# zhouhang95/ray_tracing_in_one_weekend

Hardware: AMD Instinct MI355X
Metric: Mray/s (primary+secondary) at 1920x1080/256spp (higher is better)
Workload: dtype f32

## Files before the change

include/rtow_mi355x_debug.h:

```cpp
#ifndef RTOW_MI355X_DEBUG_H
#define RTOW_MI355X_DEBUG_H

#include "rtow_mi355x.h"

#ifdef __cplusplus
extern "C" {
#endif

#define RT_FLAG_TIME_DEPTHS 4u
#define RT_FLAG_PRODUCTION_KERNELS 8u

int rt_get_depth_timings(RtCtx* ctx, uint32_t max_n, float* isect_ms, float* shade_ms, uint64_t* rays);

int rt_debug_render_parts(const RtCtx* ctx, char* buf, uint32_t cap);

enum RtDebugOption {
    RT_OPT_TREE_PLACEMENT = 0,
    RT_OPT_PRIMARY_LISTS = 1,
    RT_OPT_PIXEL_ORDER = 2,
    RT_OPT_TEXEL_POOL = 3,
    RT_OPT_GRID = 4,
    RT_OPT_GRID_CELL = 5,
    RT_OPT_CHAINS = 6,
    RT_OPT_GENERAL_KERNELS = 7,
    RT_OPT_GENERAL_LDS = 8,
    RT_OPT_QUEUE_SHARDS = 9,
    RT_OPT_ISECT_WORKGROUPS = 10,
    RT_OPT_MATERIALISE_PRIMARIES = 11,
    RT_OPT_MEDIUM_SEARCH = 12,
    RT_OPT_POOL_CHUNK_DELAY_US = 13,
    RT_OPT__COUNT = 14
};
int rt_debug_set_option(RtCtx* ctx, uint32_t option, uint32_t value);
int rt_debug_get_option(const RtCtx* ctx, uint32_t option, uint32_t* value);

typedef struct RtSceneInfo {
    uint32_t n_entries;
    uint32_t n_tree_nodes, tree_depth;
    uint32_t tree_in_lds;
    uint32_t general_kernels;
    uint32_t closest_hit_lds_bytes;
    uint32_t grid;
    uint32_t grid_cells[3];
    uint32_t grid_refs;
    uint32_t grid_always;
    uint32_t grid_lds_bytes;
    float grid_cell_size[3];
    uint32_t general_tables_in_lds;
    uint32_t nest;
} RtSceneInfo;
int rt_debug_scene_info(const RtCtx* ctx, RtSceneInfo* info);

int rt_debug_planar_info(const RtCtx* ctx, uint32_t* n_planar, uint32_t* plane_data_in_lds);
int rt_debug_planar_bounds(const RtQuads* quads, float world_mag, float* box, float* slack);

int rt_debug_grid_build(const RtFlatScene* scene, uint32_t cell_per_mille, uint32_t lds_budget, float grid[8], uint32_t dims[3],
                        uint32_t* cells, uint32_t* n_cells, uint16_t* refs, uint32_t* n_refs, uint32_t large[4], uint32_t* n_large);

int rt_debug_world_bounds(const RtFlatScene* scene, float* prim_box, float* prim_box_padded, float* world_sphere, uint32_t* n_entries,
                          uint32_t* entry_id, float* entry_box_padded, float* entry_bs);

int rt_debug_motion_bounds(const RtCtx* ctx, float* entry_box_padded, float* entry_sphere, uint32_t* entry_id, uint32_t entry_cap, uint32_t* n_entries,
                           float grid[6], uint32_t dims[3], uint32_t* cell_begin, uint32_t* cell_id, uint32_t cell_cap, uint32_t* n_cell_ids);

// ... 33 lines not shown
```

ray_tracing_in_one_weekend_amd/_ffi.py:

```python
import ctypes as C
import os

_PKG_DIR = os.path.dirname(os.path.abspath(__file__))
GPU_LIB_PATH = os.environ.get("RTOW_GPU_LIB") or os.path.join(_PKG_DIR, "librtow_mi355x.so")
HOST_LIB_PATH = os.path.join(_PKG_DIR, "librtow_host.so")

RT_NO_TEX = 0xFFFFFFFF
ERR_INVALID, ERR_DEVICE, ERR_NOMEM, ERR_UNSUPPORTED, ERR_STATE = 1, 2, 3, 4, 5
FLAG_BRUTE_FORCE = 1
FLAG_RUSSIAN_ROULETTE = 2
FLAG_TIME_DEPTHS = 4
FLAG_PRODUCTION_KERNELS = 8
RTH_INVALID = 0xFFFFFFFF

(MAT_EMISSION, MAT_DIFFUSE, MAT_LAMBERT, MAT_METAL, MAT_DIELECTRIC, MAT_ISOTROPIC, MAT_OREN_NAYAR,
 MAT_BURLEY_DIFFUSE, MAT_ROUGH_PLASTIC, MAT_DISNEY_DIFFUSE, MAT_DISNEY_METAL, MAT_DISNEY_SHEEN,
 MAT_DISNEY_CLEARCOAT) = range(13)
TEX_CONSTANT, TEX_CHECKER, TEX_PERLIN, TEX_IMAGE = range(4)
RECT_YZ, RECT_XZ, RECT_XY = range(3)
XF_TRANSLATE, XF_ROTATE_Y = range(2)
NO_XFORM = 0xFFFFFFFF
SKY_GRADIENT, SKY_BLACK, SKY_ENV = range(3)

_f = C.POINTER(C.c_float)
# ... 49 lines not shown
PLANAR_MIN_SIN2 = 2.0 ** -20
PLANAR_REACH = 16.0


class RtParams(C.Structure):
    _fields_ = [("nx", C.c_uint32), ("ny", C.c_uint32), ("spp", C.c_uint32), ("max_depth", C.c_int32),
                ("seed", C.c_uint64), ("shard_band", C.c_uint32), ("shard_count", C.c_uint32),
                ("shard_id", C.c_uint32), ("spp_slice", C.c_uint32), ("flags", C.c_uint32), ("reserved", C.c_uint32)]


class RtStats(C.Structure):
    _fields_ = [("n_paths", C.c_uint64), ("n_rays", C.c_uint64), ("n_rays_secondary", C.c_uint64),
                ("n_texture_fetches", C.c_uint64), ("n_bad_dir", C.c_uint64), ("seconds_total", C.c_double),
                ("seconds_trace", C.c_double), ("seconds_device", C.c_double), ("bytes_algorithmic", C.c_uint64),
                ("bytes_trace_algorithmic", C.c_uint64), ("n_trace_launches", C.c_uint32), ("n_slices", C.c_uint32),
                ("rays_per_depth", C.c_uint64 * 64)]

    def as_dict(self):
        d = {k: getattr(self, k) for k, _ in self._fields_ if k != "rays_per_depth"}
        d["rays_per_depth"] = list(self.rays_per_depth)
        return d


class RtBounceIO(C.Structure):
    _fields_ = [("n", C.c_uint32), ("depth", C.c_uint32), ("in_o", _f), ("in_d", _f), ("in_key", _u32),
                ("out_hit", C.POINTER(C.c_int32)), ("out_t", _f), ("out_radiance", _f), ("out_attenuation", _f),
                ("out_o", _f), ("out_d", _f), ("out_alive", _u8), ("flags", C.c_uint32)]


RtProgressFn = C.CFUNCTYPE(None, C.c_void_p, C.c_uint32, C.c_uint32, C.POINTER(C.c_uint8), C.c_uint32, C.c_uint32)

MULTI_COPY_GATHER = 1
(OPT_TREE_PLACEMENT, OPT_PRIMARY_LISTS, OPT_PIXEL_ORDER, OPT_TEXEL_POOL, OPT_GRID, OPT_GRID_CELL, OPT_CHAINS,
 OPT_GENERAL_KERNELS, OPT_GENERAL_LDS, OPT_QUEUE_SHARDS, OPT_ISECT_WORKGROUPS, OPT_MATERIALISE_PRIMARIES, OPT_MEDIUM_SEARCH, OPT_POOL_CHUNK_DELAY_US) = range(14)
OPT_NAMES = {"tree_placement": OPT_TREE_PLACEMENT, "primary_lists": OPT_PRIMARY_LISTS, "pixel_order": OPT_PIXEL_ORDER,
             "texel_pool": OPT_TEXEL_POOL, "grid": OPT_GRID, "grid_cell": OPT_GRID_CELL, "chains": OPT_CHAINS,
             "general_kernels": OPT_GENERAL_KERNELS, "general_lds": OPT_GENERAL_LDS, "queue_shards": OPT_QUEUE_SHARDS,
             "isect_workgroups": OPT_ISECT_WORKGROUPS, "materialise_primaries": OPT_MATERIALISE_PRIMARIES,
             "medium_search": OPT_MEDIUM_SEARCH, "pool_chunk_delay_us": OPT_POOL_CHUNK_DELAY_US}


class RtSceneInfo(C.Structure):
    _fields_ = [("n_entries", C.c_uint32), ("n_tree_nodes", C.c_uint32), ("tree_depth", C.c_uint32), ("tree_in_lds", C.c_uint32),
                ("general_kernels", C.c_uint32), ("closest_hit_lds_bytes", C.c_uint32), ("grid", C.c_uint32),
                ("grid_cells", C.c_uint32 * 3), ("grid_refs", C.c_uint32), ("grid_always", C.c_uint32),
                ("grid_lds_bytes", C.c_uint32), ("grid_cell_size", C.c_float * 3), ("general_tables_in_lds", C.c_uint32), ("nest", C.c_uint32)]

    def as_dict(self):
        d = {k: getattr(self, k) for k, _ in self._fields_ if k not in ("grid_cells", "grid_cell_size")}
        d["grid_cells"], d["grid_cell_size"] = list(self.grid_cells), [float(x) for x in self.grid_cell_size]
        return d


EXPECTED_ABI = 11
GPU_SYMBOLS = ["rt_abi_version", "rt_build_id", "rt_ctx_create", "rt_ctx_destroy", "rt_last_error", "rt_scene_upload",
               "rt_shard_rows", "rt_shard_row_to_image_row", "rt_prepare", "rt_render", "rt_render_device", "rt_debug_bounce", "rt_debug_arithmetic",
               "rt_get_depth_timings", "rt_set_progress", "rt_host_alloc", "rt_host_free", "rt_debug_set_option", "rt_debug_get_option",
               "rt_debug_scene_info", "rt_debug_grid_build", "rt_debug_world_bounds", "rt_debug_render_parts", "rt_multi_create", "rt_multi_create_ex", "rt_multi_destroy", "rt_multi_device_count",
               "rt_multi_last_error", "rt_multi_scene_upload", "rt_multi_render", "rt_deinterleave_bands", "rt_set_lens", "rt_multi_set_lens",
               "rt_set_motion", "rt_multi_set_motion", "rt_debug_motion_bounds",
               "rt_set_quads", "rt_multi_set_quads", "rt_debug_planar_info", "rt_debug_planar_bounds"]
HOST_SYMBOLS = ["rth_last_error", "rth_register_image", "rth_rng_reseed", "rth_scene_build", "rth_scene_new",
                "rth_tex_constant", "rth_tex_checker", "rth_tex_perlin", "rth_tex_image", "rth_material",
                "rth_sphere", "rth_rect", "rth_gbox", "rth_translate", "rth_rotate_y", "rth_constant_medium", "rth_hitable_bbox", "rth_set_sky", "rth_set_camera", "rth_scene_finish", "rth_scene_flat",
                "rth_scene_camera", "rth_scene_sphere_name", "rth_scene_free", "rth_png_write", "rth_output_file_name",
                "rth_set_camera_lens", "rth_scene_lens",
                "rth_moving_sphere", "rth_set_camera_shutter", "rth_scene_motion",
                "rth_quad", "rth_triangle", "rth_scene_quads"]

_gpu_lib = None
_host_lib = None

# ... 181 lines not shown
```

ray_tracing_in_one_weekend_amd/csrc/rt_api.hip:

```cpp
#include "../../include/rtow_mi355x_debug.h"
#include "rt_kernels.h"
#include "rt_bvh.h"
#include "rt_grid.h"
#include "rt_pool.h"

#include <hip/hip_runtime.h>

#include <algorithm>
#include <chrono>
#include <cmath>
#include <cstdio>
#include <cstdlib>
#include <cstring>
#include <new>
#include <string>
#include <vector>

using namespace rt;

namespace {

thread_local std::string g_create_error;

struct DevBuf {
// ... 1431 lines not shown
        gp.s0 = s0;
        gp.n_rays = npix * sc;
        RT_HIP(ctx, hipMemsetAsync(counts, 0, counts_bytes, st));
        if (ctx->motion) hipLaunchKernelGGL(k_set_motion, dim3(1), dim3(64), 0, st, gpd, ctx->gmotion);
        if (ctx->planar) hipLaunchKernelGGL(k_set_planar, dim3(1), dim3(64), 0, st, gpd, ctx->gplanar);
        if (lens) hipLaunchKernelGGL(k_init_counts<true>, dim3((nq + 255u) / 256u), dim3(256), 0, st, gp, counts, gpd, glens);
        else hipLaunchKernelGGL(k_init_counts<false>, dim3((nq + 255u) / 256u), dim3(256), 0, st, gp, counts, gpd, glens);
        if (!fuse_gen && lens) hipLaunchKernelGGL(k_gen_primary<true>, dim3((gp.n_rays + 255u) / 256u), dim3(256), 0, st, gp, Q[0], glens);
        else if (!fuse_gen) hipLaunchKernelGGL(k_gen_primary<false>, dim3((gp.n_rays + 255u) / 256u), dim3(256), 0, st, gp, Q[0], glens);
        RT_HIP(ctx, hipEventRecord(ctx->events[2 * sl], st));
        if (n_groups > 1u) {
            RT_HIP(ctx, hipEventRecord(ctx->ev_fork, st));
            RT_HIP(ctx, hipStreamWaitEvent(ctx->stream2, ctx->ev_fork, 0));
        }
        for (int depth = 0; depth < n_depths; ++depth)
        for (uint32_t grp = 0; grp < n_groups; ++grp) {
            hipStream_t sg = grp ? ctx->stream2 : st;
            const uint32_t q0 = grp * (nq / n_groups), q1 = grp + 1u == n_groups ? nq : q0 + nq / n_groups;
            const uint32_t isect_grid_g = (q1 - q0 + shards_per_wg - 1u) / shards_per_wg;
            const Queue& qi = Q[depth & 1];
            const Queue& qo = Q[(depth + 1) & 1];
            const uint32_t* cin = counts + (size_t)depth * nq;
            uint32_t* cout = counts + (size_t)(depth + 1) * nq;
            const bool td = time_depths && sl == 0;
            if (td) RT_HIP(ctx, hipEventRecord(ctx->depth_events[3 * (size_t)depth], st));
            const bool gen = fuse_gen && depth == 0;
            ip.depth = depth;
            ip.q0 = q0, ip.q1 = q1;
            const StepBuffers sb{qi, qo, qhit, cin, cout, rad, totals, gpd, lens, ctx->motion, ctx->planar};
            const bool no_primary_trace = gen && !rects && gp.lists != nullptr && no_overflow;
            if (!no_primary_trace) launch_intersect(ctx, sg, use_bvh, gen, isect_grid_g, sb, ip);
            if (td) RT_HIP(ctx, hipEventRecord(ctx->depth_events[3 * (size_t)depth + 1], st));
            const ShadeParams sp{nq, cap, depth, prm->max_depth, depth > 0 ? 1u : 0u,
                                 (prm->flags & RT_FLAG_RUSSIAN_ROULETTE) ? 1u : 0u, q0};
            launch_shade(ctx, sg, gen, !rects && gp.lists != nullptr, q1 - q0, sb, sp);
            if (td) RT_HIP(ctx, hipEventRecord(ctx->depth_events[3 * (size_t)depth + 2], st));
            if (grp == 0u) n_trace_launches += no_primary_trace ? 1u : 2u;
        }
        if (n_groups > 1u) {
            RT_HIP(ctx, hipEventRecord(ctx->ev_join, ctx->stream2));
            RT_HIP(ctx, hipStreamWaitEvent(st, ctx->ev_join, 0));
        }
        if (time_depths && sl == 0) {
            ctx->timed_depths = n_depths;
            ctx->timed_rays.assign((size_t)n_depths, 0ull);
            std::vector<uint32_t> hc((size_t)(n_depths + 1) * nq);
            RT_HIP(ctx, hipMemcpyAsync(hc.data(), counts, hc.size() * sizeof(uint32_t), hipMemcpyDeviceToHost, st));
            RT_HIP(ctx, hipStreamSynchronize(st));
            for (int d = 0; d < n_depths; ++d)
                for (uint32_t k = 0; k < nq; ++k) ctx->timed_rays[(size_t)d] += hc[(size_t)d * nq + k];
        }
        RT_HIP(ctx, hipEventRecord(ctx->events[2 * sl + 1], st));
        hipLaunchKernelGGL(k_resolve, dim3((npix + 255u) / 256u), dim3(256), 0, st, rad, acc, npix, sc);
        hipLaunchKernelGGL(k_accum_counts, dim3((unsigned)n_depths), dim3(256), 0, st, counts, nq, (uint32_t)n_depths, totals + 2);
        if (ctx->progress_armed && ctx->progress_fn && s0 + sc < spp) {
            const uint32_t done = s0 + sc;
            hipLaunchKernelGGL(k_finalize, dim3((npix + 255u) / 256u), dim3(256), 0, st, acc, (float*)nullptr,
                               (uint8_t*)ctx->preview_u8.p, nx, rows, done, gp.tiles_per_row, gp.tile_pixels);
            RT_HIP(ctx, hipMemcpyAsync(ctx->preview_host.data(), ctx->preview_u8.p, (size_t)npix * 3, hipMemcpyDeviceToHost, st));
            RT_HIP(ctx, hipStreamSynchronize(st));
            ctx->progress_fn(ctx->progress_user, done, spp, ctx->preview_host.data(), nx, rows);
        }
        s0 += sc;
    }
    if (pool_wait_ms > 0.0) ctx->parts.emplace_back("of_which_waiting_for_the_pool", pool_wait_ms);
    hipLaunchKernelGGL(k_finalize, dim3((npix + 255u) / 256u), dim3(256), 0, st, acc, (float*)d_out_rgb_f32,
                       (uint8_t*)d_out_rgb8, nx, rows, spp, gp.tiles_per_row, gp.tile_pixels);
// ... 673 lines not shown
    if ((rc = ensure(ctx, ctx->counts, (size_t)2 * nq * sizeof(uint32_t)))) return rc;
    if ((rc = ensure(ctx, ctx->totals, 4 * sizeof(unsigned long long)))) return rc;
    if ((rc = ensure(ctx, ctx->genp, sizeof(GenParams) + RT_PLANAR_OFFSET + sizeof(GenPlanar)))) return rc;
    if ((rc = ensure(ctx, ctx->dbg, (size_t)n * 6 * sizeof(float)))) return rc;
    const WorkLayout wl = work_layout((size_t)nq * cap, n);
    const size_t wbase = work_base(ctx);
    if (const char* e = pool_request(ctx->pool, wbase + wl.total)) return fail(ctx, RT_ERR_NOMEM, std::string("rt_debug_bounce: ") + e);
    if (!pool_wait(ctx->pool, wbase + wl.total)) return fail(ctx, RT_ERR_NOMEM, "rt_debug_bounce: no device memory for the work buffers: " + pool_error(ctx->pool));
    const WorkView wv = work_view(ctx, wl, wbase);
    const Queue* Q = wv.Q;
    uint32_t* counts = (uint32_t*)ctx->counts.p;
    float* d_o = (float*)ctx->dbg.p;
    float* d_d = d_o + 3 * (size_t)n;
    RT_HIP(ctx, hipMemcpyAsync(d_o, io->in_o, 3 * (size_t)n * 4, hipMemcpyHostToDevice, st));
    RT_HIP(ctx, hipMemcpyAsync(d_d, io->in_d, 3 * (size_t)n * 4, hipMemcpyHostToDevice, st));
    RT_HIP(ctx, hipMemsetAsync(counts, 0, (size_t)2 * nq * sizeof(uint32_t), st));
    RT_HIP(ctx, hipMemsetAsync(ctx->totals.p, 0, 4 * sizeof(unsigned long long), st));
    RT_HIP(ctx, hipMemsetAsync(wv.rad, 0xFF, (size_t)n * RT_RAD_FLOATS * sizeof(float), st));
    GenParams gp{};
    gp.nx = n, gp.ny = 1, gp.npix = n, gp.n_rays = n, gp.s0 = 0;
    gp.shard_band = 1, gp.shard_count = 1, gp.shard_id = 0;
    gp.nq = nq, gp.cap = cap;
    gp.inv_npix = gp.inv_nx = (float)((1.0 / (double)n) * (1.0 - 1.0 / 4194304.0));
    gp.inv_band = (float)(1.0 - 1.0 / 4194304.0);
    hipLaunchKernelGGL(k_init_counts<false>, dim3((nq + 255u) / 256u), dim3(256), 0, st, gp, counts, (GenParams*)ctx->genp.p, GenLens{});
    if (ctx->motion) hipLaunchKernelGGL(k_set_motion, dim3(1), dim3(64), 0, st, (GenParams*)ctx->genp.p, ctx->gmotion);
    if (ctx->planar) hipLaunchKernelGGL(k_set_planar, dim3(1), dim3(64), 0, st, (GenParams*)ctx->genp.p, ctx->gplanar);
    hipLaunchKernelGGL(k_debug_fill, dim3((n + 255u) / 256u), dim3(256), 0, st, gp, Q[0], d_o, d_d);
    const bool use_bvh = ctx->use_bvh && !(io->flags & RT_FLAG_BRUTE_FORCE);
    const StepBuffers sb{Q[0], Q[1], wv.qhit, counts, counts + nq, wv.rad,
                         (unsigned long long*)ctx->totals.p, (const GenParams*)ctx->genp.p, false, ctx->motion, ctx->planar};
    const IntersectParams ip{nq, cap, (int)io->depth, 0u, nq};
    launch_intersect(ctx, st, use_bvh, false, qg.isect_grid, sb, ip);
    const ShadeParams sp{nq, cap, (int)io->depth, 0x7FFFFFFF, 1u, 0u, 0u};
    launch_shade(ctx, st, false, false, nq, sb, sp);
    RT_HIP(ctx, hipGetLastError());
    std::vector<float4> ha((size_t)nq * cap), hb((size_t)nq * cap);
    std::vector<float> hrad((size_t)n * RT_RAD_FLOATS);
    std::vector<float2> hc((size_t)nq * cap), hh((size_t)nq * cap);
    std::vector<uint32_t> hcnt((size_t)2 * nq);
    RT_HIP(ctx, hipMemcpyAsync(hh.data(), wv.qhit, hh.size() * sizeof(float2), hipMemcpyDeviceToHost, st));
    std::vector<float4> hab;
    if (RT_QSTRIDE == 1u) {
        RT_HIP(ctx, hipMemcpyAsync(ha.data(), Q[1].a, ha.size() * sizeof(float4), hipMemcpyDeviceToHost, st));
        RT_HIP(ctx, hipMemcpyAsync(hb.data(), Q[1].b, hb.size() * sizeof(float4), hipMemcpyDeviceToHost, st));
    } else {
        hab.resize(2 * ha.size());
        RT_HIP(ctx, hipMemcpyAsync(hab.data(), Q[1].a, hab.size() * sizeof(float4), hipMemcpyDeviceToHost, st));
    }
    RT_HIP(ctx, hipMemcpyAsync(hc.data(), Q[1].c, hc.size() * sizeof(float2), hipMemcpyDeviceToHost, st));
    RT_HIP(ctx, hipMemcpyAsync(hrad.data(), wv.rad, hrad.size() * sizeof(float), hipMemcpyDeviceToHost, st));
    RT_HIP(ctx, hipMemcpyAsync(hcnt.data(), counts, hcnt.size() * sizeof(uint32_t), hipMemcpyDeviceToHost, st));
    RT_HIP(ctx, hipStreamSynchronize(st));
    for (size_t i = 0; i < hab.size() / 2; ++i) ha[i] = hab[2 * i], hb[i] = hab[2 * i + 1];
    auto bits = [](float f) {
        uint32_t u;
        std::memcpy(&u, &f, 4);
        return u;
    };
    for (uint32_t i = 0; i < n; ++i) {
        const uint32_t chunk = i >> 8;
        const size_t pos = (size_t)(chunk % nq) * cap + (size_t)(chunk / nq) * 256u + (i & 255u);
        const int hit = (int)bits(hh[pos].y);
        io->out_hit[i] = hit;
        io->out_t[i] = hit >= 0 ? hh[pos].x : 0.0f;
        io->out_alive[i] = 0;
        for (int k = 0; k < 3; ++k) io->out_attenuation[3 * (size_t)i + k] = io->out_o[3 * (size_t)i + k] = io->out_d[3 * (size_t)i + k] = 0.0f;
// ... 125 lines not shown
```

ray_tracing_in_one_weekend_amd/csrc/rt_device.h:

```cpp
#pragma once
#include <hip/hip_runtime.h>
#include <stdint.h>

namespace rt {

struct V3 {
    float x, y, z;
};
struct V2 {
    float x, y;
};
__device__ __forceinline__ V3 v3(float x, float y, float z) { return V3{x, y, z}; }
__device__ __forceinline__ V3 splat(float s) { return V3{s, s, s}; }
__device__ __forceinline__ V3 operator+(V3 a, V3 b) { return V3{a.x + b.x, a.y + b.y, a.z + b.z}; }
__device__ __forceinline__ V3 operator-(V3 a, V3 b) { return V3{a.x - b.x, a.y - b.y, a.z - b.z}; }
__device__ __forceinline__ V3 operator*(V3 a, V3 b) { return V3{a.x * b.x, a.y * b.y, a.z * b.z}; }
__device__ __forceinline__ V3 operator/(V3 a, V3 b) { return V3{a.x / b.x, a.y / b.y, a.z / b.z}; }
__device__ __forceinline__ V3 operator*(V3 a, float s) { return V3{a.x * s, a.y * s, a.z * s}; }
__device__ __forceinline__ V3 operator*(float s, V3 a) { return V3{s * a.x, s * a.y, s * a.z}; }
__device__ __forceinline__ V3 operator/(V3 a, float s) { return V3{a.x / s, a.y / s, a.z / s}; }
__device__ __forceinline__ V3 operator+(V3 a, float s) { return V3{a.x + s, a.y + s, a.z + s}; }
__device__ __forceinline__ V3 operator-(float s, V3 a) { return V3{s - a.x, s - a.y, s - a.z}; }
__device__ __forceinline__ V3 operator-(V3 a) { return V3{-a.x, -a.y, -a.z}; }
__device__ __forceinline__ float dot(V3 a, V3 b) { return (a.x * b.x + a.y * b.y) + a.z * b.z; }
// ... 68 lines not shown
#define RT_LANE_STAT(I, PRED)                                                                      \
    do {                                                                                           \
        const unsigned long long act_ = __ballot(true), m_ = __ballot(PRED);                       \
        if ((threadIdx.x & 63u) == (uint32_t)__ffsll((long long)act_) - 1u) {                      \
            atomicAdd(&g_lane_stats[I], 64ull);                                                    \
            atomicAdd(&g_lane_stats[(I) + 1], (unsigned long long)__popcll(m_));                   \
        }                                                                                          \
    } while (0)
#else
#define RT_LANE_STAT(I, PRED)
#endif

__device__ __forceinline__ uint32_t fmix32(uint32_t h) {
    h ^= h >> 16;
    h *= 0x85EBCA6Bu;
    h ^= h >> 13;
    h *= 0xC2B2AE35u;
    h ^= h >> 16;
    return h;
}
__device__ __forceinline__ uint32_t mix32(uint32_t h) {
    h ^= h >> 16;
    h *= 0x7FEB352Du;
    h ^= h >> 15;
    h *= 0x846CA68Bu;
    h ^= h >> 16;
    return h;
}
__device__ __forceinline__ void path_key(uint64_t seed, uint32_t pix, uint32_t samp, uint32_t& k0, uint32_t& k1) {
    uint32_t s_lo = (uint32_t)seed, s_hi = (uint32_t)(seed >> 32);
    uint32_t a = fmix32(pix ^ s_lo);
    k0 = fmix32(a + samp * 0x9E3779B9u + s_hi);
    k1 = fmix32((a ^ 0xA511E9B3u) + samp * 0xC2B2AE3Du);
}
struct Rng {
    uint32_t k0, k1, w;
    __device__ __forceinline__ Rng() {}
    __device__ __forceinline__ Rng(uint32_t k0_, uint32_t k1_, uint32_t ctr) : k0(k0_), k1(k1_), w(ctr * 0x9E3779B9u) {}
    __device__ __forceinline__ float next() {
        uint32_t r = mix32((k0 ^ w) + k1);
        w += 0x9E3779B9u;
        return (float)(r >> 8) * (1.0f / 16777216.0f);
    }
    __device__ __forceinline__ float next_pm1() {
        uint32_t r = mix32((k0 ^ w) + k1);
        w += 0x9E3779B9u;
        return __builtin_fmaf((float)(r >> 8), 1.0f / 8388608.0f, -1.0f);
    }
};
__device__ __forceinline__ uint32_t depth_counter_base(int depth) { return (uint32_t)(depth + 1) * 256u; }

__device__ __forceinline__ V3 random_in_unit_sphere(Rng& rng) {
    RT_LANE_STAT(10, true);
    for (;;) {
        RT_LANE_STAT(8, true);
        const float x = rng.next_pm1();
        const float y = rng.next_pm1();
        const float z = rng.next_pm1();
        const V3 v = v3(x, y, z);
        if (length_squared(v) < 1.0f) return v;
    }
}
__device__ __forceinline__ V3 random_on_hemisphere(Rng& rng, V3 n) {
    V3 v = random_in_unit_sphere(rng);
    if (!(dot(v, n) > 0.0f)) v = -v;
    return normalize(v);
// ... 278 lines not shown
    V3 oc = o - v3(g.x, g.y, g.z);
    float half_b = dot(oc, d);
    float c = length_squared(oc) - g.w * g.w;
    if (t_min > 0.0f && half_b > 0.0f && c > 0.0f) return false;
    float discriminant = half_b * half_b - a * c;
    if (discriminant < 0.0f) return false;
    float sqrtd = sqrt_ns(discriminant);
    float root = (-half_b - sqrtd) / a;
    if (root < t_min || t_max < root) {
        root = (-half_b + sqrtd) / a;
        if (root < t_min || t_max < root) return false;
    }
    t_hit = root;
    return true;
}

__device__ __forceinline__ bool sphere_root(float4 g, V3 o, V3 d, const SharedRcp& ra, float t_min, float t_max, float& t_hit) {
    V3 oc = o - v3(g.x, g.y, g.z);
    float half_b = dot(oc, d);
    float c = length_squared(oc) - g.w * g.w;
    if (half_b > 0.0f && c > 0.0f) return false;
    float discriminant = half_b * half_b - ra.a * c;
    if (discriminant < 0.0f) return false;
    float sqrtd = sqrt_ns(discriminant);
    float root = div_shared(-half_b - sqrtd, ra);
    if (root < t_min || t_max < root) {
        root = div_shared(-half_b + sqrtd, ra);
        if (root < t_min || t_max < root) return false;
    }
    t_hit = root;
    return true;
}

__device__ __forceinline__ bool rect_root(float4 g0, float4 g1, V3 o, V3 d, float t_min, float t_max, float& t_hit) {
    const uint32_t axis = __float_as_uint(g1.y);
    const float oa = axis == 0u ? o.x : (axis == 1u ? o.y : o.z);
    const float da = axis == 0u ? d.x : (axis == 1u ? d.y : d.z);
    const float t = (g0.x - oa) / da;
    if (!(t == t) || t < t_min || t > t_max) return false;
    const V3 p = o + d * t;
    const float pu = axis == 0u ? p.y : p.x;
    const float pv = axis == 2u ? p.y : p.z;
    if (pu < g0.y || pu > g0.z || pv < g0.w || pv > g1.x) return false;
    t_hit = t;
    return true;
}

#define RT_PLANAR_TRIANGLE_DEV 1u
__device__ __forceinline__ void planar_coords(const float4* __restrict__ g, V3 P, float& alpha, float& beta) {
    const float4 q4 = g[1], u4 = g[2], v4 = g[3], w4 = g[4];
    const V3 p = P - v3(q4.x, q4.y, q4.z);
    const V3 w = v3(w4.x, w4.y, w4.z);
    alpha = dot(w, cross(p, v3(v4.x, v4.y, v4.z)));
    beta = dot(w, cross(v3(u4.x, u4.y, u4.z), p));
}
__device__ __forceinline__ bool planar_root(const float4* __restrict__ g, V3 o, V3 d, float t_min, float t_max, float& t_hit) {
    const float4 nd = g[0];
    const V3 normal = v3(nd.x, nd.y, nd.z);
    const float denom = dot(normal, d);
    if (fabsf(denom) < 1e-8f) return false;
    const float t = (nd.w - dot(normal, o)) / denom;
    if (!(t == t) || t < t_min || t > t_max) return false;
    const V3 P = o + d * t;
    float alpha, beta;
    planar_coords(g, P, alpha, beta);
    const bool inside = __float_as_uint(g[1].w) == RT_PLANAR_TRIANGLE_DEV ? (alpha >= 0.0f && beta >= 0.0f && alpha + beta <= 1.0f)
// ... 371 lines not shown
```

ray_tracing_in_one_weekend_amd/csrc/rt_kernels.h:

```cpp
#pragma once
#include "rt_device.h"

namespace rt {

#ifndef RT_QSTRIDE
#define RT_QSTRIDE 2u
#endif
struct Queue {
    float4* a;
    float4* b;
    float2* c;
};
#ifndef RT_RAD_FLOATS
#define RT_RAD_FLOATS 3
#endif
__device__ __forceinline__ void rad_store(float* __restrict__ rad, size_t slot, float x, float y, float z) {
    if (RT_RAD_FLOATS == 4) *reinterpret_cast<float4*>(rad + 4u * slot) = make_float4(x, y, z, 0.0f);
    else *reinterpret_cast<float3*>(rad + 3u * slot) = make_float3(x, y, z);
}

struct GenParams {
    float cam_origin[3], cam_horizontal[3], cam_vertical[3], cam_llc[3];
    uint32_t nx, ny;
    uint32_t npix;
// ... 97 lines not shown
    Rng rng;
    path_key(((uint64_t)gp.seed_hi << 32) | gp.seed_lo, j * gp.nx + i, samp, rng.k0, rng.k1);
    rng.w = 0u;
    const float u = ((float)i + rng.next()) / (float)gp.nx;
    const float v = ((float)j + rng.next()) / (float)gp.ny;
    const V3 origin = v3(gp.cam_origin[0], gp.cam_origin[1], gp.cam_origin[2]);
    const V3 H = v3(gp.cam_horizontal[0], gp.cam_horizontal[1], gp.cam_horizontal[2]);
    const V3 Vv = v3(gp.cam_vertical[0], gp.cam_vertical[1], gp.cam_vertical[2]);
    const V3 llc = v3(gp.cam_llc[0], gp.cam_llc[1], gp.cam_llc[2]);
    o = origin;
    if (!LENS) {
        d = normalize(llc + u * H + v * Vv - origin);
    } else {
        const V3 dir = llc + u * H + v * Vv - origin;
        float rx = 0.0f, ry = 0.0f;
        for (uint32_t t = 0; t < RT_LENS_TRIPS; ++t) {
            const float x = rng.next_pm1(), y = rng.next_pm1();
            if (x * x + y * y < 1.0f) {
                rx = x, ry = y;
                break;
            }
        }
        const V3 off = rx * v3(gl.lu[0], gl.lu[1], gl.lu[2]) + ry * v3(gl.lv[0], gl.lv[1], gl.lv[2]);
        o = origin + off;
        d = normalize(gl.focus_dist * dir - off);
    }
    k0 = rng.k0, k1 = rng.k1;
}
template <bool LENS>
__device__ __forceinline__ void gen_primary(const GenParams& gp, const GenLens& gl, uint32_t idx, V3& o, V3& d, uint32_t& k0,
                                            uint32_t& k1) {
    uint32_t pl;
    gen_primary<LENS>(gp, gl, idx, o, d, k0, k1, pl);
}

__device__ __forceinline__ uint32_t primary_idx_of(uint32_t nq, uint32_t shard, uint32_t pos) {
    return ((pos >> 8) * nq + shard) * 256u + (pos & 255u);
}
template <bool LENS>
__global__ __launch_bounds__(256) void k_init_counts(GenParams gp, uint32_t* __restrict__ counts,
                                                     GenParams* __restrict__ gp_dev, GenLens gl) {
    const uint32_t sq = blockIdx.x * 256u + threadIdx.x;
    if (sq == 0) *gp_dev = gp;
    if (LENS && sq == 0) *reinterpret_cast<GenLens*>(gp_dev + 1) = gl;
    if (sq >= gp.nq) return;
    const uint32_t nchunks = (gp.n_rays + 255u) / 256u;
    const uint32_t nc = sq < nchunks ? (nchunks - sq + gp.nq - 1u) / gp.nq : 0u;
    uint32_t cnt = nc * 256u;
    if (nc && ((nchunks - 1u) % gp.nq) == sq) cnt -= nchunks * 256u - gp.n_rays;
    counts[sq] = cnt;
}

__global__ void k_set_motion(GenParams* __restrict__ gp_dev, GenMotion gm) {
    if (blockIdx.x == 0 && threadIdx.x == 0) *reinterpret_cast<GenMotion*>(reinterpret_cast<char*>(gp_dev + 1) + RT_MOTION_OFFSET) = gm;
}

__global__ void k_set_planar(GenParams* __restrict__ gp_dev, GenPlanar pl) {
    if (blockIdx.x == 0 && threadIdx.x == 0) *reinterpret_cast<GenPlanar*>(reinterpret_cast<char*>(gp_dev + 1) + RT_PLANAR_OFFSET) = pl;
}

template <bool LENS>
__global__ __launch_bounds__(256) void k_gen_primary(GenParams gp, Queue q, GenLens gl) {
    const uint32_t idx = blockIdx.x * 256u + threadIdx.x;
    if (idx >= gp.n_rays) return;
    V3 o, d;
    uint32_t k0, k1;
// ... 818 lines not shown
            tbest = th;
            hit = (int)(gq.base + i);
        }
    }
}

__global__ __launch_bounds__(256) void k_intersect_list_planar(DevScene sc, const float4* __restrict__ qa, const float4* __restrict__ qb,
                                                               float2* __restrict__ qh, const uint32_t* __restrict__ in_counts,
                                                               IntersectParams ip, const GenParams* __restrict__ gpd) {
    const uint32_t q = ip.q0 + blockIdx.x;
    const uint32_t count = in_counts[q];
    const size_t qbase = (size_t)q * ip.cap;
    const GenPlanar gq = gen_planar_of(gpd);
    for (uint32_t i = threadIdx.x; i < count; i += 256u) {
        const float4 ra = qa[RT_QSTRIDE * (qbase + i)], rb = qb[RT_QSTRIDE * (qbase + i)];
        const V3 o = v3(ra.x, ra.y, ra.z), d = v3(rb.x, rb.y, rb.z);
        float tbest = RT_FLT_MAX;
        int hit = -1;
        closest_hit_spheres_general(sc, o, d, tbest, hit);
        MediumCtx mc{0u, 0u, depth_counter_base(ip.depth)};
        if (sc.n_media) path_key_of_slot(*gpd, __float_as_uint(ra.w), mc.k0, mc.k1);
        closest_hit_rects(sc, o, d, mc, tbest, hit);
        closest_hit_planar(gq, o, d, tbest, hit);
        qh[qbase + i] = make_float2(tbest, __int_as_float(hit));
    }
}

struct ShadeParams {
    uint32_t nq, cap;
    int depth, max_depth;
    uint32_t sort;
    uint32_t russian_roulette;
    uint32_t q0;
};

#ifdef RT_PROFILE_PHASES
__device__ unsigned long long g_phase_stats[16];
#define RT_PHASE_CLOCK() __builtin_amdgcn_s_memtime()
#else
#define RT_PHASE_CLOCK() 0ull
#endif

#define RT_PERLIN_LDS_MAX_SETS 4u
#ifndef RT_SORT_N
#define RT_SORT_N 512u
#endif
#define RT_NCLASS 64u
#define RT_CLASS_LDS_MAX 4096u
#define RT_SHADE_WAVE_LDS (RT_NCLASS * 4u + RT_SORT_N * 8u + RT_SORT_N * 2u)
__host__ __device__ inline size_t shade_lds_bytes(uint32_t n_entries, uint32_t n_perlin_lds, uint32_t n_fused_spheres, bool sort) {
    size_t b = 16u;
    if (sort) b += 4u * RT_SHADE_WAVE_LDS;
    if (sort && n_entries <= RT_CLASS_LDS_MAX) b += ((size_t)n_entries + 15u) & ~(size_t)15u;
    b += (size_t)n_perlin_lds * (4096u + 1536u);
    b += (size_t)n_fused_spheres * 16u;
    return (b + 15u) & ~(size_t)15u;
}
template <bool PERLIN_LDS, bool GEN, bool RECTS, bool NEST = false, bool LENS = false, bool MOTION = false, bool PLANAR = false>
#ifndef RT_GEN_WAVES
#define RT_GEN_WAVES 4
#endif
#ifndef RT_SORTED_WAVES
#define RT_SORTED_WAVES 4
#endif
__global__ __launch_bounds__(256, GEN ? RT_GEN_WAVES : RT_SORTED_WAVES) void k_shade(DevScene sc, Queue qin, const float2* __restrict__ qh, Queue qout,
                                               const uint32_t* __restrict__ in_counts, uint32_t* __restrict__ out_counts,
// ... 3 lines not shown
    extern __shared__ __attribute__((aligned(16))) char smem[];
    const uint32_t q = tp.q0 + blockIdx.x;
    const uint32_t count = in_counts[q];
    if (count == 0) return;
    uint32_t* s_out = reinterpret_cast<uint32_t*>(smem);
    const uint32_t lane = threadIdx.x & 63u;
    const uint32_t w = __builtin_amdgcn_readfirstlane(threadIdx.x >> 6);
    const bool sort = !GEN && tp.sort != 0u;
    size_t lds_off = 16u;
    uint32_t* s_hist = reinterpret_cast<uint32_t*>(smem + lds_off + (size_t)w * RT_SHADE_WAVE_LDS);
    float2* s_rec = reinterpret_cast<float2*>(s_hist + RT_NCLASS);
    unsigned short* s_pos = reinterpret_cast<unsigned short*>(s_rec + RT_SORT_N);
    const uint8_t* cls = sc.sph_class;
    if (sort) {
        lds_off += 4u * RT_SHADE_WAVE_LDS;
        const uint32_t n_ent = sc.n_prims + sc.n_media + (PLANAR ? gen_planar_of(gpd).n : 0u);
        if (n_ent <= RT_CLASS_LDS_MAX) {
            uint8_t* lc = reinterpret_cast<uint8_t*>(smem + lds_off);
            for (uint32_t i = threadIdx.x; i < n_ent; i += 256u) lc[i] = sc.sph_class[i];
            cls = lc;
            lds_off += ((size_t)n_ent + 15u) & ~(size_t)15u;
        }
    }
    PerlinTables pt{sc.perlin_vec, sc.perlin_perm2};
    if (PERLIN_LDS) {
        float4* lv = reinterpret_cast<float4*>(smem + lds_off);
        unsigned short* lp = reinterpret_cast<unsigned short*>(lv + sc.n_perlin * 256u);
        for (uint32_t i = threadIdx.x; i < sc.n_perlin * 256u; i += 256u) lv[i] = sc.perlin_vec[i];
        for (uint32_t i = threadIdx.x; i < sc.n_perlin * 768u; i += 256u) lp[i] = sc.perlin_perm2[i];
        pt = PerlinTables{lv, lp};
        lds_off += (size_t)sc.n_perlin * (4096u + 1536u);
    }
    const bool fused = GEN && !RECTS && gpd->lists != nullptr;
    const float4* s_geo = reinterpret_cast<const float4*>(smem + lds_off);
    if (fused) {
        float4* g = reinterpret_cast<float4*>(smem + lds_off);
        for (uint32_t i = threadIdx.x; i < sc.n_spheres; i += 256u) g[i] = sc.sph_geo[i];
        if (MOTION)
            for (uint32_t i = threadIdx.x; i < sc.n_spheres; i += 256u) g[sc.n_spheres + i] = gen_motion_of(gpd).sph_dc[i];
    }
    const float4* s_dc = s_geo + sc.n_spheres;
    if (threadIdx.x == 0) *s_out = 0u;
    __syncthreads();
    uint32_t n_fetch = 0, n_bad = 0;
    const size_t qbase = (size_t)q * tp.cap;
#ifdef RT_PROFILE_PHASES
    unsigned long long ph[10] = {};
    const unsigned long long ph_t0 = RT_PHASE_CLOCK();
#endif
    const uint32_t bs = count >= 4u * RT_SORT_N ? RT_SORT_N : ((count + 255u) / 256u) * 64u;
    for (uint32_t base = w * bs; base < count; base += 4u * bs) {
        const uint32_t n_here = min(bs, count - base);
#ifdef RT_PROFILE_PHASES
        const unsigned long long ph_a0 = RT_PHASE_CLOCK();
        asm volatile("s_waitcnt vmcnt(0)" ::: "memory");
        const unsigned long long ph_a = RT_PHASE_CLOCK();
        ph[8] += ph_a - ph_a0;
#endif
        if (sort) {
            s_hist[lane] = 0u;
            __builtin_amdgcn_fence(__ATOMIC_ACQ_REL, "workgroup");
            float2 h[RT_SORT_N / 64u];
            uint32_t kr[RT_SORT_N / 64u];
            __builtin_amdgcn_s_waitcnt(0x0F70);
#pragma unroll
            for (uint32_t k = 0; k < RT_SORT_N / 64u; ++k) {
                const uint32_t j = k * 64u + lane;
                h[k] = j < n_here ? qh[qbase + base + j] : make_float2(0.0f, 0.0f);
            }
#ifdef RT_PROFILE_PHASES
// ... 58 lines not shown
#endif
        for (uint32_t seg = 0; seg < n_here; seg += 64u) {
            float2 hB = make_float2(0.0f, 0.0f), rcB = hB;
            float4 raB = make_float4(0.f, 0.f, 0.f, 0.f), rbB = raB;
            bool prefetched = false;
            auto prefetch = [&]() {
                if (!prefetched && seg + 64u < n_here) fetch(seg + 64u, hB, raB, rbB, rcB);
                prefetched = true;
            };
            const uint32_t j = seg + lane;
            RT_LANE_STAT(18, j < n_here);
            if (!GEN && __all(j >= n_here || __float_as_int(hA.y) < 0)) {
                if (j < n_here) {
                    const V3 d = v3(rbA.x, rbA.y, rbA.z);
                    V3 Lr = splat(0.0f);
                    if (!near_one(d)) ++n_bad;
                    else Lr = v3(rbA.w, rcA.x, rcA.y) * sky_value(sc, d, n_fetch);
                    rad_store(rad, __float_as_uint(raA.w), Lr.x, Lr.y, Lr.z);
                }
                prefetch();
                hA = hB, raA = raB, rbA = rbB, rcA = rcB;
#ifdef RT_PROFILE_PHASES
                { const unsigned long long t = RT_PHASE_CLOCK(); ph[3] += t - ph_c, ph[6] += 1, ph_c = t; }
#endif
                continue;
            }
            bool alive = false;
            Bounce bo;
            bo.o = bo.d = bo.attenuation = splat(0.0f);
            V3 T = splat(0.0f);
            float rr_threshold = 0.0f;
            uint32_t slot = 0, k0 = 0, k1 = 0;
            float tm = 0.0f;
            if (j < n_here) {
                float2 h = hA;
                V3 o, d;
                if (GEN) {
                    uint32_t pl;
                    slot = primary_idx_of(tp.nq, q, base + j);
                    gen_primary<LENS>(*gpd, gen_lens_of(gpd), slot, o, d, k0, k1, pl);
                    if (MOTION) tm = path_time(gen_motion_of(gpd), k0, k1);
                    T = splat(1.0f);
                    uint4 list = make_uint4(RT_LIST_OVERFLOW, 0u, 0u, 0u);
                    if (fused) list = gpd->lists[pl];
                    const uint32_t n_list = list.x & 0xFFFFu;
                    RT_LANE_STAT(14, fused && n_list != RT_LIST_OVERFLOW);
                    if (fused && n_list != RT_LIST_OVERFLOW) {
                        const SharedRcp ra = shared_rcp(length_squared(d));
                        float tbest = RT_FLT_MAX;
                        int hit = -1;
                        const uint32_t ids[RT_LIST_MAX] = {list.x >> 16, list.y & 0xFFFFu, list.y >> 16, list.z & 0xFFFFu,
                                                           list.z >> 16, list.w & 0xFFFFu, list.w >> 16};
#pragma unroll
                        for (uint32_t t = 0; t < RT_LIST_MAX; ++t) {
                            float th;
                            const int s = (int)ids[t];
                            if (t < n_list) RT_LANE_STAT(12, true);
                            if (t < n_list && sphere_root(MOTION ? sphere_at(s_geo[s], s_dc[s], tm) : s_geo[s], o, d, ra, 1e-3f, RT_FLT_MAX, th) &&
                                (th < tbest || (th == tbest && s > hit))) {
                                tbest = th;
                                hit = s;
                            }
                        }
                        h = make_float2(tbest, __int_as_float(hit));
                    } else {
                        h = qh[qbase + base + j];
                    }
                } else {
                    o = v3(raA.x, raA.y, raA.z), d = v3(rbA.x, rbA.y, rbA.z);
                    T = v3(rbA.w, rcA.x, rcA.y);
                    slot = __float_as_uint(raA.w);
                    path_key_of_slot(*gpd, slot, k0, k1);
                    if (MOTION) tm = path_time(gen_motion_of(gpd), k0, k1);
                }
                V3 Lr = splat(0.0f);
                if (!near_one(d)) {
                    ++n_bad;
                } else {
#ifdef RT_DEBUG_QUEUE_BOUNDS
                    if (__float_as_int(h.y) >= (int)(sc.n_prims + sc.n_media + (PLANAR ? gen_planar_of(gpd).n : 0u))) __builtin_trap();
#endif
                    Rng rng{k0, k1, depth_counter_base(tp.depth)};
                    bo = shade<RECTS, decltype(prefetch), NEST, MOTION, PLANAR>(sc, pt, o, d, __float_as_int(h.y), h.x, rng, n_fetch, prefetch,
                                                                                MOTION ? gen_motion_of(gpd).sph_dc : nullptr, tm,
                                                                                PLANAR ? gen_planar_of(gpd).pq : nullptr,
                                                                                PLANAR ? gen_planar_of(gpd).base : 0u);
                    if (bo.alive && tp.russian_roulette) {
                        const float rr = rng.next();
                        rr_threshold = fmaxf(bo.attenuation.x, fmaxf(bo.attenuation.y, bo.attenuation.z));
                        if (!(rr < rr_threshold)) bo.alive = false;
                    }
// ... 313 lines not shown
```

Measured before the change: 30810.

## Share per-wavefront primary-ray setup and precompute sphere-origin terms in depth-0 shading

For pinhole, non-motion sphere scenes with fused primary lists, the shade kernel now precomputes per-sphere origin offsets and c terms once into LDS, since all primary rays share the camera origin. It also computes tile coordinates and sample key terms once per wavefront using uniform reciprocal division and readfirstlane, instead of a full per-lane index decomposition. This removes redundant integer divisions, hashing and sphere setup per primary ray, at the cost of extra code paths and registers. The path is on by default (per_lane is 0 unless the option is set to 1) and changes the floating-point evaluation order slightly.

Result: slower. 29760 (-3.4%).

```diff
diff --git a/include/rtow_mi355x_debug.h b/include/rtow_mi355x_debug.h
--- a/include/rtow_mi355x_debug.h
+++ b/include/rtow_mi355x_debug.h
@@ -29,7 +29,8 @@
     RT_OPT_MATERIALISE_PRIMARIES = 11,
     RT_OPT_MEDIUM_SEARCH = 12,
     RT_OPT_POOL_CHUNK_DELAY_US = 13,
-    RT_OPT__COUNT = 14
+    RT_OPT_DEPTH0_SHARED_WORK = 14,
+    RT_OPT__COUNT = 15
 };
 int rt_debug_set_option(RtCtx* ctx, uint32_t option, uint32_t value);
 int rt_debug_get_option(const RtCtx* ctx, uint32_t option, uint32_t* value);
diff --git a/ray_tracing_in_one_weekend_amd/_ffi.py b/ray_tracing_in_one_weekend_amd/_ffi.py
--- a/ray_tracing_in_one_weekend_amd/_ffi.py
+++ b/ray_tracing_in_one_weekend_amd/_ffi.py
@@ -105,12 +105,14 @@
 
 MULTI_COPY_GATHER = 1
 (OPT_TREE_PLACEMENT, OPT_PRIMARY_LISTS, OPT_PIXEL_ORDER, OPT_TEXEL_POOL, OPT_GRID, OPT_GRID_CELL, OPT_CHAINS,
- OPT_GENERAL_KERNELS, OPT_GENERAL_LDS, OPT_QUEUE_SHARDS, OPT_ISECT_WORKGROUPS, OPT_MATERIALISE_PRIMARIES, OPT_MEDIUM_SEARCH, OPT_POOL_CHUNK_DELAY_US) = range(14)
+ OPT_GENERAL_KERNELS, OPT_GENERAL_LDS, OPT_QUEUE_SHARDS, OPT_ISECT_WORKGROUPS, OPT_MATERIALISE_PRIMARIES, OPT_MEDIUM_SEARCH, OPT_POOL_CHUNK_DELAY_US,
+ OPT_DEPTH0_SHARED_WORK) = range(15)
 OPT_NAMES = {"tree_placement": OPT_TREE_PLACEMENT, "primary_lists": OPT_PRIMARY_LISTS, "pixel_order": OPT_PIXEL_ORDER,
              "texel_pool": OPT_TEXEL_POOL, "grid": OPT_GRID, "grid_cell": OPT_GRID_CELL, "chains": OPT_CHAINS,
              "general_kernels": OPT_GENERAL_KERNELS, "general_lds": OPT_GENERAL_LDS, "queue_shards": OPT_QUEUE_SHARDS,
              "isect_workgroups": OPT_ISECT_WORKGROUPS, "materialise_primaries": OPT_MATERIALISE_PRIMARIES,
-             "medium_search": OPT_MEDIUM_SEARCH, "pool_chunk_delay_us": OPT_POOL_CHUNK_DELAY_US}
+             "medium_search": OPT_MEDIUM_SEARCH, "pool_chunk_delay_us": OPT_POOL_CHUNK_DELAY_US,
+             "depth0_shared_work": OPT_DEPTH0_SHARED_WORK}
 
 
 class RtSceneInfo(C.Structure):
diff --git a/ray_tracing_in_one_weekend_amd/csrc/rt_api.hip b/ray_tracing_in_one_weekend_amd/csrc/rt_api.hip
--- a/ray_tracing_in_one_weekend_amd/csrc/rt_api.hip
+++ b/ray_tracing_in_one_weekend_amd/csrc/rt_api.hip
@@ -1487,7 +1487,7 @@
             if (!no_primary_trace) launch_intersect(ctx, sg, use_bvh, gen, isect_grid_g, sb, ip);
             if (td) RT_HIP(ctx, hipEventRecord(ctx->depth_events[3 * (size_t)depth + 1], st));
             const ShadeParams sp{nq, cap, depth, prm->max_depth, depth > 0 ? 1u : 0u,
-                                 (prm->flags & RT_FLAG_RUSSIAN_ROULETTE) ? 1u : 0u, q0};
+                                 (prm->flags & RT_FLAG_RUSSIAN_ROULETTE) ? 1u : 0u, q0, ctx->opt[RT_OPT_DEPTH0_SHARED_WORK] == 1u ? 1u : 0u};
             launch_shade(ctx, sg, gen, !rects && gp.lists != nullptr, q1 - q0, sb, sp);
             if (td) RT_HIP(ctx, hipEventRecord(ctx->depth_events[3 * (size_t)depth + 2], st));
             if (grp == 0u) n_trace_launches += no_primary_trace ? 1u : 2u;
@@ -2227,7 +2227,7 @@
                          (unsigned long long*)ctx->totals.p, (const GenParams*)ctx->genp.p, false, ctx->motion, ctx->planar};
     const IntersectParams ip{nq, cap, (int)io->depth, 0u, nq};
     launch_intersect(ctx, st, use_bvh, false, qg.isect_grid, sb, ip);
-    const ShadeParams sp{nq, cap, (int)io->depth, 0x7FFFFFFF, 1u, 0u, 0u};
+    const ShadeParams sp{nq, cap, (int)io->depth, 0x7FFFFFFF, 1u, 0u, 0u, 0u};
     launch_shade(ctx, st, false, false, nq, sb, sp);
     RT_HIP(ctx, hipGetLastError());
     std::vector<float4> ha((size_t)nq * cap), hb((size_t)nq * cap);
diff --git a/ray_tracing_in_one_weekend_amd/csrc/rt_device.h b/ray_tracing_in_one_weekend_amd/csrc/rt_device.h
--- a/ray_tracing_in_one_weekend_amd/csrc/rt_device.h
+++ b/ray_tracing_in_one_weekend_amd/csrc/rt_device.h
@@ -124,6 +124,11 @@
     uint32_t a = fmix32(pix ^ s_lo);
     k0 = fmix32(a + samp * 0x9E3779B9u + s_hi);
     k1 = fmix32((a ^ 0xA511E9B3u) + samp * 0xC2B2AE3Du);
+}
+__device__ __forceinline__ void path_key_terms(uint32_t s_lo, uint32_t pix, uint32_t ka, uint32_t kb, uint32_t& k0, uint32_t& k1) {
+    uint32_t a = fmix32(pix ^ s_lo);
+    k0 = fmix32(a + ka);
+    k1 = fmix32((a ^ 0xA511E9B3u) + kb);
 }
 struct Rng {
     uint32_t k0, k1, w;
@@ -468,6 +473,28 @@
     return true;
 }
 
+__device__ __forceinline__ float4 sphere_from_origin(float4 g, V3 o) {
+    V3 oc = o - v3(g.x, g.y, g.z);
+    float c = length_squared(oc) - g.w * g.w;
+    return make_float4(oc.x, oc.y, oc.z, c);
+}
+__device__ __forceinline__ bool sphere_root_from_origin(float4 s, V3 d, const SharedRcp& ra, float t_min, float t_max, float& t_hit) {
+    V3 oc = v3(s.x, s.y, s.z);
+    float half_b = dot(oc, d);
+    float c = s.w;
+    if (half_b > 0.0f && c > 0.0f) return false;
+    float discriminant = half_b * half_b - ra.a * c;
+    if (discriminant < 0.0f) return false;
+    float sqrtd = sqrt_ns(discriminant);
+    float root = div_shared(-half_b - sqrtd, ra);
+    if (root < t_min || t_max < root) {
+        root = div_shared(-half_b + sqrtd, ra);
+        if (root < t_min || t_max < root) return false;
+    }
+    t_hit = root;
+    return true;
+}
+
 __device__ __forceinline__ bool rect_root(float4 g0, float4 g1, V3 o, V3 d, float t_min, float t_max, float& t_hit) {
     const uint32_t axis = __float_as_uint(g1.y);
     const float oa = axis == 0u ? o.x : (axis == 1u ? o.y : o.z);
diff --git a/ray_tracing_in_one_weekend_amd/csrc/rt_kernels.h b/ray_tracing_in_one_weekend_amd/csrc/rt_kernels.h
--- a/ray_tracing_in_one_weekend_amd/csrc/rt_kernels.h
+++ b/ray_tracing_in_one_weekend_amd/csrc/rt_kernels.h
@@ -153,6 +153,65 @@
                                             uint32_t& k1) {
     uint32_t pl;
     gen_primary<LENS>(gp, gl, idx, o, d, k0, k1, pl);
+}
+
+__device__ __forceinline__ uint32_t udiv_inv_uniform(uint32_t x, uint32_t d, float inv, uint32_t& rem) {
+    uint32_t qt = __builtin_amdgcn_readfirstlane((uint32_t)((float)x * inv));
+    uint32_t r = x - qt * d;
+    if (r >= d) ++qt, r -= d;
+    if (r >= d) ++qt, r -= d;
+    rem = r;
+    return qt;
+}
+struct PrimaryTile {
+    uint32_t i0, lj0;
+    uint32_t pl0;
+    uint32_t pix0;
+    uint32_t jbase, rb0;
+    uint32_t ka, kb;
+};
+__device__ __forceinline__ bool primary_tile_of(const GenParams& gp, uint32_t idx0, PrimaryTile& t) {
+    if (gp.tiles_per_row == 0u || (gp.npix & 63u) != 0u || (gp.shard_count > 1u && gp.shard_band < 8u)) return false;
+    const uint32_t s_local = udiv_inv_uniform(idx0, gp.npix, gp.inv_npix, t.pl0);
+    if (t.pl0 >= gp.tile_pixels) return false;
+    uint32_t tx;
+    const uint32_t ty = udiv_inv_uniform(t.pl0 >> 6, gp.tiles_per_row, gp.inv_tpr, tx);
+    t.i0 = tx * 8u, t.lj0 = ty * 8u;
+    t.pix0 = t.lj0 * gp.nx + t.i0;
+    t.jbase = 0u, t.rb0 = 0u;
+    if (gp.shard_count > 1u) {
+        const uint32_t bq = udiv_inv_uniform(t.lj0, gp.shard_band, gp.inv_band, t.rb0);
+        t.jbase = (bq * gp.shard_count + gp.shard_id) * gp.shard_band;
+    }
+    const uint32_t samp = gp.s0 + s_local;
+    t.ka = samp * 0x9E3779B9u + gp.seed_hi, t.kb = samp * 0xC2B2AE3Du;
+    return true;
+}
+__device__ __forceinline__ void gen_primary_tile(const GenParams& gp, const PrimaryTile& t, uint32_t lane, uint32_t lane_pix, const SharedRcp& rnx,
+                                                 const SharedRcp& rny, V3& o, V3& d, uint32_t& k0, uint32_t& k1, uint32_t& pl) {
+    const uint32_t i = t.i0 + (lane & 7u);
+    uint32_t j, pix;
+    if (gp.shard_count > 1u) {
+        const uint32_t rb = t.rb0 + (lane >> 3);
+        j = t.jbase + rb + (rb >= gp.shard_band ? (gp.shard_count - 1u) * gp.shard_band : 0u);
+        pix = j * gp.nx + i;
+    } else {
+        j = t.lj0 + (lane >> 3);
+        pix = t.pix0 + lane_pix;
+    }
+    pl = t.pl0 + lane;
+    Rng rng;
+    path_key_terms(gp.seed_lo, pix, t.ka, t.kb, rng.k0, rng.k1);
+    rng.w = 0u;
+    const float u = div_shared((float)i + rng.next(), rnx);
+    const float v = div_shared((float)j + rng.next(), rny);
+    const V3 origin = v3(gp.cam_origin[0], gp.cam_origin[1], gp.cam_origin[2]);
+    const V3 H = v3(gp.cam_horizontal[0], gp.cam_horizontal[1], gp.cam_horizontal[2]);
+    const V3 Vv = v3(gp.cam_vertical[0], gp.cam_vertical[1], gp.cam_vertical[2]);
+    const V3 llc = v3(gp.cam_llc[0], gp.cam_llc[1], gp.cam_llc[2]);
+    o = origin;
+    d = normalize(llc + u * H + v * Vv - origin);
+    k0 = rng.k0, k1 = rng.k1;
 }
 
 __device__ __forceinline__ uint32_t primary_idx_of(uint32_t nq, uint32_t shard, uint32_t pos) {
@@ -1037,6 +1096,7 @@
     uint32_t sort;
     uint32_t russian_roulette;
     uint32_t q0;
+    uint32_t per_lane;
 };
 
 #ifdef RT_PROFILE_PHASES
@@ -1106,10 +1166,21 @@
         lds_off += (size_t)sc.n_perlin * (4096u + 1536u);
     }
     const bool fused = GEN && !RECTS && gpd->lists != nullptr;
+    constexpr bool SHARED = GEN && !RECTS && !LENS && !MOTION && !PLANAR;
+    const bool shared = SHARED && tp.per_lane == 0u;
+    const GenParams gp = GEN ? *gpd : GenParams{};
+    SharedRcp rnx{1.0f, 1.0f}, rny{1.0f, 1.0f};
+    uint32_t lane_pix = 0u;
+    if (SHARED) rnx = shared_rcp((float)gp.nx), rny = shared_rcp((float)gp.ny), lane_pix = (lane >> 3) * gp.nx + (lane & 7u);
     const float4* s_geo = reinterpret_cast<const float4*>(smem + lds_off);
     if (fused) {
         float4* g = reinterpret_cast<float4*>(smem + lds_off);
-        for (uint32_t i = threadIdx.x; i < sc.n_spheres; i += 256u) g[i] = sc.sph_geo[i];
+        if (shared) {
+            const V3 origin = v3(gp.cam_origin[0], gp.cam_origin[1], gp.cam_origin[2]);
+            for (uint32_t i = threadIdx.x; i < sc.n_spheres; i += 256u) g[i] = sphere_from_origin(sc.sph_geo[i], origin);
+        } else {
+            for (uint32_t i = threadIdx.x; i < sc.n_spheres; i += 256u) g[i] = sc.sph_geo[i];
+        }
         if (MOTION)
             for (uint32_t i = threadIdx.x; i < sc.n_spheres; i += 256u) g[sc.n_spheres + i] = gen_motion_of(gpd).sph_dc[i];
     }
@@ -1234,17 +1305,21 @@
             float rr_threshold = 0.0f;
             uint32_t slot = 0, k0 = 0, k1 = 0;
             float tm = 0.0f;
+            PrimaryTile pt0{};
+            bool tile = false;
+            if (SHARED && shared) tile = primary_tile_of(gp, __builtin_amdgcn_readfirstlane(primary_idx_of(tp.nq, q, base + seg)), pt0);
             if (j < n_here) {
                 float2 h = hA;
                 V3 o, d;
                 if (GEN) {
                     uint32_t pl;
                     slot = primary_idx_of(tp.nq, q, base + j);
-                    gen_primary<LENS>(*gpd, gen_lens_of(gpd), slot, o, d, k0, k1, pl);
+                    if (SHARED && tile) gen_primary_tile(gp, pt0, lane, lane_pix, rnx, rny, o, d, k0, k1, pl);
+                    else gen_primary<LENS>(gp, gen_lens_of(gpd), slot, o, d, k0, k1, pl);
                     if (MOTION) tm = path_time(gen_motion_of(gpd), k0, k1);
                     T = splat(1.0f);
                     uint4 list = make_uint4(RT_LIST_OVERFLOW, 0u, 0u, 0u);
-                    if (fused) list = gpd->lists[pl];
+                    if (fused) list = gp.lists[pl];
                     const uint32_t n_list = list.x & 0xFFFFu;
                     RT_LANE_STAT(14, fused && n_list != RT_LIST_OVERFLOW);
                     if (fused && n_list != RT_LIST_OVERFLOW) {
@@ -1258,7 +1333,9 @@
                             float th;
                             const int s = (int)ids[t];
                             if (t < n_list) RT_LANE_STAT(12, true);
-                            if (t < n_list && sphere_root(MOTION ? sphere_at(s_geo[s], s_dc[s], tm) : s_geo[s], o, d, ra, 1e-3f, RT_FLT_MAX, th) &&
+                            if (t < n_list &&
+                                (shared ? sphere_root_from_origin(s_geo[s], d, ra, 1e-3f, RT_FLT_MAX, th)
+                                        : sphere_root(MOTION ? sphere_at(s_geo[s], s_dc[s], tm) : s_geo[s], o, d, ra, 1e-3f, RT_FLT_MAX, th)) &&
                                 (th < tbest || (th == tbest && s > hit))) {
                                 tbest = th;
                                 hit = s;
```
